# Rutgers-ECE-MML4SS/multimodal-sensor-fusion-with-attention-RajeevAtla

Hardware: AMD Instinct MI355X
Metric: HybridFusion fwd+bwd samples/sec at 1/2/4/8 MI355X; CPU-ref parity (higher is better)
Workload: dtype fp32; 1 GPU; c2: HybridFusion M=3 B=256/gpu L=128 D=128 H=128 heads=4 C=5 dropout=0.1 train, fwd+CE(ls=0.05)+bwd+clip(1.0)+AdamW; fused step (flat buffers, one hipGraph); global_batch=256, per_gpu_batch=256, seq_len=128, parallelism=dp1, graph=True, matmul_precision=highest

## Files before the change

### include/mmfusion.h

```cpp
#ifndef MMFUSION_H_
#define MMFUSION_H_

#include <stddef.h>
#include <stdint.h>

#ifdef __cplusplus
extern "C" {
#endif

#define MMF_MAX_MODALITIES 8
#define MMF_MAX_PAIRS (MMF_MAX_MODALITIES * (MMF_MAX_MODALITIES - 1))
#define MMF_MAX_HEAD_DIM 64

enum {
  MMF_PRECISION_HIGHEST = 0,
  MMF_PRECISION_MEDIUM = 1,
  MMF_PRECISION_HIGH = 2
};

enum {
  MMF_OK = 0,
  MMF_EINVAL = 1,
  MMF_ELIMIT = 2,
  MMF_EHIP = 3,
// ... 200 lines not shown
size_t mmf_transformer_encoder_saved_bytes(int32_t batch, int32_t steps, int32_t hidden, int32_t ffn,
                                           int32_t layers);
size_t mmf_transformer_encoder_workspace_bytes(int32_t batch, int32_t steps, int32_t hidden, int32_t ffn,
                                               int32_t layers, int32_t backward);
int mmf_transformer_encoder_forward(const mmf_transformer_desc* desc, const mmf_transformer_layer* params,
                                    const float* x, const int64_t* lengths, uint64_t* rng_state, void* saved,
                                    float* pooled, void* workspace, void* stream);
int mmf_transformer_encoder_backward(const mmf_transformer_desc* desc, const mmf_transformer_layer* params,
                                     const float* x, const int64_t* lengths, const void* saved,
                                     const float* dpooled, void* workspace,
                                     const mmf_transformer_layer_grad* grads, float* dx, void* stream);

int mmf_cross_entropy_ls(int32_t batch, int32_t classes, const float* logits,
                         const int64_t* labels, float smoothing, float grad_scale,
                         float* loss_out, float* dlogits, void* stream);

int mmf_adamw_step(int64_t n, float* param, const float* grad, float* exp_avg, float* exp_avg_sq,
                   int64_t* step_dev, float lr, float beta1, float beta2, float eps,
                   float weight_decay, float grad_scale, void* stream);

size_t mmf_hybrid_train_sync_bytes(const mmf_hybrid_desc* d);
int mmf_hybrid_lean_l1(const mmf_hybrid_desc* d);
int mmf_hybrid_train_status(const mmf_hybrid_desc* d, void* sync, int clear, void* stream);
int mmf_hybrid_train_step(const mmf_hybrid_desc* d, const mmf_hybrid_params* params, const float* const* x,
                          const float* mask, const int64_t* labels, float label_smoothing, float loss_scale,
                          uint64_t* rng_state, void* saved, void* workspace, void* sync, float* logits,
                          float* fusion_weights, float* loss_out, float* dlogits, const mmf_hybrid_grads* grads,
                          float* const* dx, float* clip_partial, int64_t* step_dev, const float* grad_flat,
                          int64_t grad_n, void* stream);

int mmf_hybrid_train_step_part(int part, const mmf_hybrid_desc* d, const mmf_hybrid_params* params,
                               const float* const* x, const float* mask, const int64_t* labels,
                               float label_smoothing, float loss_scale, uint64_t* rng_state, void* saved,
                               void* workspace, void* sync, float* logits, float* fusion_weights, float* loss_out,
                               float* dlogits, const mmf_hybrid_grads* grads, float* const* dx, float* clip_partial,
                               int64_t* step_dev, const float* grad_flat, int64_t grad_n, void* stream);

int mmf_adamw_step_dev(int64_t n, float* param, const float* grad, float* exp_avg, float* exp_avg_sq,
                       int64_t* step_dev, const float* lr_dev, const float* grad_coef_dev, float beta1,
                       float beta2, float eps, float weight_decay, float grad_scale, void* stream);

int mmf_clip_adamw_apply_dev(int64_t n, float* param, const float* grad, float* exp_avg, float* exp_avg_sq,
                             int64_t* step_dev, const float* lr_dev, float max_norm, float* total_norm,
                             float* clip_coef, void* workspace, float beta1, float beta2, float eps,
                             float weight_decay, float grad_scale, void* stream);

int mmf_grad_accumulate(int64_t n, const float* src, float* dst, void* stream);

size_t mmf_gemm_bf16_workspace_bytes(int32_t M, int32_t N, int32_t K, int32_t nsplit);
int mmf_gemm_bf16(int32_t M, int32_t N, int32_t K, const void* A, int32_t lda, int32_t a_kmajor, const void* B,
                  int32_t ldb, int32_t b_kmajor, const float* bias, void* C, int32_t ldc, int32_t c_bf16,
                  void* workspace, int32_t nsplit, float* bias_grad, void* stream);

size_t mmf_grad_clip_workspace_bytes(void);
int mmf_grad_clip_coef(int64_t n, const float* grad, float grad_scale, float max_norm, float* total_norm,
                       float* clip_coef, void* workspace, void* stream);

int mmf_clip_adamw_step_dev(int64_t n, float* param, const float* grad, float* exp_avg, float* exp_avg_sq,
                            int64_t* step_dev, const float* lr_dev, float max_norm, float* total_norm,
                            float* clip_coef, void* workspace, float beta1, float beta2, float eps,
                            float weight_decay, float grad_scale, void* stream);

void mmf_profile_begin(void);
size_t mmf_profile_end(char* out, size_t cap);

const char* mmf_last_error(void);
const char* mmf_version(void);

#ifdef __cplusplus
}
#endif
#endif
```

### multimodal-sensor-fusion-with-attention-rajeevatla_amd/csrc/capi.hip

```cpp
#include <cmath>
#include <map>

#include "capi_util.h"

namespace mmf {

thread_local std::string g_err;
Prof g_prof;

int fail(int code, const char* fmt, ...) {
  char buf[512];
  va_list ap;
  va_start(ap, fmt);
  vsnprintf(buf, sizeof(buf), fmt, ap);
  va_end(ap);
  g_err = buf;
  return code;
}

}

using namespace mmf;

namespace {
// ... 491 lines not shown
  hipStream_t st = (hipStream_t)stream;
  STAGE_TRY("optim.clip_adamw", launch_clip_adamw_apply(n, param, grad, exp_avg, exp_avg_sq, step_dev, lr_dev, beta1,
                                                        beta2, eps, weight_decay, grad_scale, max_norm, total_norm,
                                                        clip_coef, (const float*)workspace, st));
  return MMF_OK;
}

int mmf_grad_accumulate(int64_t n, const float* src, float* dst, void* stream) {
  if (n < 0 || (n > 0 && (!src || !dst))) return fail(MMF_EINVAL, "bad gradient-accumulate arguments");
  if ((reinterpret_cast<uintptr_t>(src) | reinterpret_cast<uintptr_t>(dst)) & 15)
    return fail(MMF_EINVAL, "gradient accumulate: buffers must be 16-byte aligned");
  hipStream_t st = (hipStream_t)stream;
  STAGE_TRY("optim.grad_accum", launch_grad_accum(n, src, dst, st));
  return MMF_OK;
}

size_t mmf_gemm_bf16_workspace_bytes(int32_t M, int32_t N, int32_t K, int32_t nsplit) {
  if (M < 1 || N < 1 || K < 1 || nsplit < 1) return 0;
  int ns = nsplit, kchunk = 0;
  split_rows(K, ns, kchunk, nsplit);
  return ((((size_t)ns * M * N * 4) + 255) & ~size_t(255)) + ((((size_t)ns * M * 4) + 255) & ~size_t(255)) + 256;
}

int mmf_gemm_bf16(int32_t M, int32_t N, int32_t K, const void* A, int32_t lda, int32_t a_kmajor, const void* B,
                  int32_t ldb, int32_t b_kmajor, const float* bias, void* C, int32_t ldc, int32_t c_bf16,
                  void* workspace, int32_t nsplit, float* bias_grad, void* stream) {
  if (M < 1 || N < 1 || K < 1 || !A || !B || !C || ldc < N || nsplit < 1)
    return fail(MMF_EINVAL, "bad bf16 GEMM arguments");
  if (a_kmajor && !b_kmajor) return fail(MMF_EINVAL, "bf16 GEMM: A k-major needs B k-major");
  if ((nsplit > 1 || bias_grad) && (!workspace || !a_kmajor || bias || c_bf16))
    return fail(MMF_EINVAL, "bf16 GEMM: split-K / bias rows need a workspace, a k-major A and an fp32 C");
  const int amode = a_kmajor ? MODE_KR : MODE_RK, bmode = b_kmajor ? MODE_KR : MODE_RK;
  hipStream_t st = (hipStream_t)stream;
  const Operand a = opnd(static_cast<const float*>(A), lda), b = opnd(static_cast<const float*>(B), ldb);
  if (nsplit == 1 && !bias_grad) {
    GemmJob j = make_job(M, N, static_cast<float*>(C), ldc, (bias ? EPI_BIAS : 0) | (c_bf16 ? EPI_BF16 : 0));
    j.g.bias = bias;
    add_src(j, a, b, K);
    if (!gemm_b16_ok(j, amode, bmode)) return fail(MMF_EINVAL, "bf16 GEMM: operand alignment / extents");
    STAGE_TRY("gemm_bf16", launch_gemm_b16(&j, 1, st, amode, bmode));
    return MMF_OK;
  }
  if (ldc != N) return fail(MMF_EINVAL, "bf16 GEMM: split-K writes a dense C (ldc == N)");
  WgradPlan wp;
  wp.split_hint = nsplit;
  Bump bw(workspace);
  plan_wgrad(wp, bw, M, N, K, a, b, static_cast<float*>(C), bias_grad, bias_grad != nullptr);
  if (!gemm_b16_ok(wp.jobs[0], amode, bmode)) return fail(MMF_EINVAL, "bf16 GEMM: operand alignment / extents");
  STAGE_TRY("gemm_bf16", launch_gemm_b16(wp.jobs.data(), 1, st, amode, bmode));
  STAGE_TRY("gemm_bf16_reduce", launch_reduce(wp.reds.data(), 1, st));
  return MMF_OK;
}

int mmf_adamw_step_dev(int64_t n, float* param, const float* grad, float* exp_avg, float* exp_avg_sq,
                       int64_t* step_dev, const float* lr_dev, const float* grad_coef_dev, float beta1,
                       float beta2, float eps, float weight_decay, float grad_scale, void* stream) {
  if (n < 0 || !param || !grad || !exp_avg || !exp_avg_sq || !step_dev || !lr_dev)
    return fail(MMF_EINVAL, "bad AdamW arguments");
  hipStream_t st = (hipStream_t)stream;
  STAGE_TRY("optim.adamw", launch_adamw(n, param, grad, exp_avg, exp_avg_sq, step_dev, 0.f, beta1, beta2, eps,
                                        weight_decay, grad_scale, st, lr_dev, grad_coef_dev));
  return MMF_OK;
}

}
```

### multimodal-sensor-fusion-with-attention-rajeevatla_amd/csrc/gemm.hip

```cpp
#include <algorithm>
#include <cstdlib>
#include <cstring>
#include <map>
#include <vector>

#include "mmf_device.h"
#include "mmf_env.h"

namespace mmf {

namespace {

constexpr int BM = 128, BN = 128, BK = 32, NT = 256;
#ifndef MMF_GEMM_DK
#define MMF_GEMM_DK 16
#endif
#ifndef MMF_GEMM_NS
#define MMF_GEMM_NS 3
#endif
constexpr int LDS_STRIDE = BM + 4;
constexpr int LDS_STRIDE_T = BM + 1;

typedef float f32x4 __attribute__((ext_vector_type(4)));

// ... 803 lines not shown
#pragma unroll
          for (int e = 0; e < 4; ++e) {
            v[e] = acc[a][b][4 * q + e] * G.alpha + bias[b];
            if (G.epi & EPI_RELU) v[e] = fmaxf(v[e], 0.f);
          }
          {
            const bool up = (x & 2) != 0;
            const float s0 = dpp<DPP_XOR2>(up ? v[0] : v[2]);
            const float s1 = dpp<DPP_XOR2>(up ? v[1] : v[3]);
            if (up) { v[0] = s0; v[1] = s1; } else { v[2] = s0; v[3] = s1; }
          }
          {
            const bool odd = (x & 1) != 0;
            const float s0 = dpp<DPP_XOR1>(odd ? v[0] : v[1]);
            const float s1 = dpp<DPP_XOR1>(odd ? v[2] : v[3]);
            if (odd) { v[0] = s0; v[2] = s1; } else { v[1] = s0; v[3] = s1; }
          }
          const int row = i0 + a * 32 + 8 * q + 4 * h + x;
          const int col = wn * 64 + b * 32 + (c & ~3);
          if (epi & EPI_ROWSCALE) {
#pragma unroll
            for (int e = 0; e < 4; ++e) v[e] *= rsc;
          }
          if (drop) {
            const uint4 rr = philox_block(rs, G.drop_site, ((uint64_t)row * (uint64_t)G.N + (uint64_t)(col & ~7)) >> 3);
#pragma unroll
            for (int e = 0; e < 4; ++e) v[e] = keep_from(rr, (col & 4) + e, thr) ? v[e] * inv_keep : 0.f;
          }
          if (epi & EPI_COLSUM) {
#pragma unroll
            for (int e = 0; e < 4; ++e) csum[b][e] += v[e];
          }
          *reinterpret_cast<f32x4*>(G.C + (int64_t)row * G.ldc + col) = f32x4{v[0], v[1], v[2], v[3]};
        }
      }
    if (epi & EPI_COLSUM) {
      float mine = 0.f;
#pragma unroll
      for (int b = 0; b < 2; ++b)
#pragma unroll
        for (int e = 0; e < 4; ++e) {
          float sv = csum[b][e];
          sv += dpp<DPP_XOR1>(sv);
          sv += dpp<DPP_XOR2>(sv);
          sv = sum_xor32(sv);
          if (b == h && e == x) mine = sv;
        }
      const int colx = wn * 64 + 32 * h + c;
      if (wm == 1) csx[colx] = mine;
      lds_barrier();
      if (wm == 0 && colx < G.N) G.colsum[(int64_t)rt * G.N + colx] = mine + csx[colx];
    }
    epi_mark = nissued;
  }
}

constexpr int WSR16_NKS = 16;
typedef __bf16 bf16x4s __attribute__((ext_vector_type(4)));

template <int WSR16_NS, int NWV = 4>
__global__ __launch_bounds__(64 * NWV, NWV == 8 ? 1 : 2) void gemm_wsr_b16_kernel(const GemmArgs args, int total_items, int K) {
  constexpr int DTILE = BM * 32 / 2;
  constexpr int PW = BM * 32 * 2 / 1024 / NWV;
  __shared__ __attribute__((aligned(16))) float ring[WSR16_NS * DTILE];
  const int t = threadIdx.x;
  const int lane = t & 63, wave = t >> 6;
  const int h = lane >> 5, c = lane & 31;
  const int wm = NWV == 8 ? wave >> 2 : wave >> 1, wn = NWV == 8 ? wave & 3 : wave & 1;
  const int nkt = K / 32, nks = K / 16;

  const int nwg = gridDim.x;
  const int item0 = (int)(((int64_t)blockIdx.x * total_items) / nwg);
  const int item1 = (int)(((int64_t)(blockIdx.x + 1) * total_items) / nwg);
  if (item0 >= item1) return;

  const int nflat = (item1 - item0) * nkt;
  auto item_group = [&](int item, int& rowtile) {
    int g = 0;
#pragma unroll
    for (int i = 1; i < GEMM_MAX_GROUPS; ++i)
      if (i < args.ngroups && item >= args.tile_off[i]) g = i;
    rowtile = item - args.tile_off[g];
    return g;
  };
  int di = item0, dk = 0, drt = 0;
  int dg = item_group(item0, drt);
  const int g_first = dg, rt_first = drt;
  auto issue = [&](int f) {
    const int slot = f % WSR16_NS;
    const GemmSrc& S = args.s[args.g[dg].src_begin];
    stage_tile_b16_nw<NWV>(ring + slot * DTILE, S.a, 0, drt * BM, args.g[dg].M, dk * 32, K, wave, lane);
    if (++dk == nkt) {
      dk = 0;
      ++di;
      ++drt;
      while (dg + 1 < args.ngroups && di >= args.tile_off[dg + 1]) { ++dg; drt = di - args.tile_off[dg]; }
    }
  };
  auto wait_ahead = [&](int ahead, bool stores_younger) {
    const int n = PW * ahead + (stores_younger ? 16 : 0);
    switch (n) {
#define MMF_WC(N) case N: asm volatile("s_waitcnt vmcnt(" #N ")" ::: "memory"); break;
      MMF_WC(0) MMF_WC(1) MMF_WC(2) MMF_WC(3) MMF_WC(4) MMF_WC(5) MMF_WC(6) MMF_WC(7) MMF_WC(8)
      MMF_WC(9) MMF_WC(10) MMF_WC(11) MMF_WC(12) MMF_WC(13) MMF_WC(14) MMF_WC(15) MMF_WC(16) MMF_WC(17)
      MMF_WC(18) MMF_WC(19) MMF_WC(20) MMF_WC(21) MMF_WC(22) MMF_WC(23) MMF_WC(24) MMF_WC(25) MMF_WC(26)
      MMF_WC(27) MMF_WC(28) MMF_WC(29) MMF_WC(30) MMF_WC(31) MMF_WC(32) MMF_WC(33) MMF_WC(34) MMF_WC(35)
// ... 509 lines not shown
hipError_t launch_wsr(const GemmJob* jobs, int njobs, hipStream_t st, uint64_t* rng_advance, int bmode, float drop_p,
                      const RngSnap* rng) {
  for (int done = 0; done < njobs;) {
    GemmArgs args;
    memset(&args, 0, sizeof(args));
    args.amode = MODE_RK;
    args.bmode = bmode;
    args.drop_p = drop_p;
    args.rng = rng;
    args.rng_advance = rng_advance;
    rng_advance = nullptr;
    int ng = 0, items = 0;
    double fl = 0.0, by = 0.0;
    while (done < njobs && ng < GEMM_MAX_GROUPS) {
      GemmGroup g = jobs[done].g;
      g.nbatch = 1;
      g.src_begin = ng;
      g.src_count = 1;
      args.s[ng] = jobs[done].src[0];
      args.tile_off[ng] = items;
      args.g[ng++] = g;
      items += g.M / BM;
      fl += 2.0 * g.M * g.N * jobs[done].src[0].K;
      by += 4.0 * ((double)g.M + g.N) * jobs[done].src[0].K + 4.0 * g.M * g.N;
      ++done;
    }
    args.ngroups = ng;
    const int K = args.s[0].K;
    const int grid = std::min(items, 2 * cu_count());
    const int pr = math_mode();
    bool ext = bmode != MODE_RK;
    for (int i = 0; i < ng; ++i) ext = ext || (args.g[i].epi & ~(EPI_BIAS | EPI_RELU)) != 0;
#define MMF_WSR_LAUNCH(BFV, EXTV, NAME)                                             \
  {                                                                                 \
    ProfLaunch prof_(st, NAME, fl, by);                                             \
    mmf_launch((gemm_wsr_kernel<BFV, EXTV>), dim3(grid), dim3(NT), 0, st, args, items, K); \
  }
    if (ext) {
      if (pr == 2) MMF_WSR_LAUNCH(2, true, "gemm_wsr_kernel<2, true>")
      else if (pr == 1) MMF_WSR_LAUNCH(1, true, "gemm_wsr_kernel<1, true>")
      else MMF_WSR_LAUNCH(0, true, "gemm_wsr_kernel<0, true>")
    } else {
      if (pr == 2) MMF_WSR_LAUNCH(2, false, "gemm_wsr_kernel<2>")
      else if (pr == 1) MMF_WSR_LAUNCH(1, false, "gemm_wsr_kernel<1>")
      else MMF_WSR_LAUNCH(0, false, "gemm_wsr_kernel<0>")
    }
#undef MMF_WSR_LAUNCH
    hipError_t e = hipGetLastError();
    if (e != hipSuccess) return e;
  }
  return hipSuccess;
}

}

int device_cu_count() { return cu_count(); }

hipError_t launch_gemm(const GemmJob* jobs_in, int njobs, int amode, int bmode, float drop_p,
                       const RngSnap* rng, hipStream_t st, uint64_t* rng_advance) {
  for (int i = 0; i < njobs; ++i)
    if ((jobs_in[i].g.epi & EPI_BF16) &&
        (!job_fast(jobs_in[i], amode, bmode) || jobs_in[i].g.nbatch > 1 || (jobs_in[i].g.epi & EPI_PARTIAL)))
      return hipErrorInvalidValue;
  {
    bool wsr = njobs > 0;
    for (int i = 0; i < njobs && wsr; ++i)
      wsr = job_wsr(jobs_in[i], amode, bmode) && jobs_in[i].src[0].K == jobs_in[0].src[0].K && !jobs_in[i].chain;
    if (wsr && !switch_set<SW_NO_WSR>()) return launch_wsr(jobs_in, njobs, st, rng_advance, bmode, drop_p, rng);
  }
  struct AdvanceLeft {
    uint64_t*& adv;
    hipStream_t st;
    hipError_t finish(hipError_t e) { return (e == hipSuccess && adv) ? launch_rng_advance(adv, st) : e; }
  } left{rng_advance, st};
  std::vector<GemmJob> rest;
  {
    SmallSlabArgs sa;
    memset(&sa, 0, sizeof(sa));
    int total = 0;
    double fl = 0.0, by = 0.0;
    auto flush = [&]() -> hipError_t {
      if (sa.ngroups == 0) return hipSuccess;
      sa.off[sa.ngroups] = total;
      ProfLaunch prof_(st, "small_slab_kernel", fl, by);
      mmf_launch(small_slab_kernel, dim3((8 * total + 255) / 256), dim3(256), 0, st, sa);
      memset(&sa, 0, sizeof(sa));
      total = 0; fl = by = 0.0;
      return hipGetLastError();
    };
    for (int i = 0; i < njobs; ++i) {
      const GemmJob& J = jobs_in[i];
      if (job_fast(J, amode, bmode) || !job_small_slab(J, amode, bmode) || J.chain) {
        rest.push_back(J);
        continue;
      }
      GemmGroup g = J.g;
      if (g.nbatch < 1) g.nbatch = 1;
      sa.g[sa.ngroups] = g;
      sa.s[sa.ngroups] = J.src[0];
      sa.off[sa.ngroups] = total;
      total += g.nbatch * g.nsplit * g.M * (g.N + (g.part_db ? 1 : 0));
      fl += 2.0 * g.nbatch * g.M * g.N * J.src[0].K;
      by += 4.0 * g.nbatch * ((double)g.M + g.N) * J.src[0].K + 4.0 * g.nbatch * g.nsplit * g.M * g.N;
      if (++sa.ngroups == GEMM_MAX_GROUPS)
        if (hipError_t e = flush()) return e;
    }
    if (hipError_t e = flush()) return e;
    if (rest.empty()) return left.finish(hipSuccess);
    jobs_in = rest.data();
    njobs = (int)rest.size();
  }
  auto chain_ok = [&](const GemmJob& J) {
    const GemmJob* C = J.chain;
    if (!C || amode != MODE_RK) return false;
    const GemmGroup &a = J.g, &b = C->g;
    if (!job_fast(J, amode, bmode) || !job_fast(*C, amode, bmode)) return false;
    if ((a.epi & (EPI_PARTIAL | EPI_BF16)) || (b.epi & EPI_PARTIAL) || a.nbatch > 1 || b.nbatch > 1) return false;
    if (a.N > BN || b.N > BN || b.M != a.M || C->nsrc != 1) return false;
    const GemmSrc& x = C->src[0];
    return x.a.ptr == a.C && x.a.ld == a.ldc && x.K == a.N && x.a.row_div == 1 && x.a.seg_stride == 0;
  };
// ... 478 lines not shown
```

### multimodal-sensor-fusion-with-attention-rajeevatla_amd/csrc/mmf_env.h

```cpp
#pragma once

#include <cstdint>
#include <cstdlib>
#include <cstring>
#include <unistd.h>

namespace mmf {

#define MMF_SWITCHES(X)        \
  X(PSTORE, 1, 0)              \
  X(NO_LONG_FUSED, 1, 0)       \
  X(NO_FUSED_BWD, 1, 0)        \
  X(NO_BF16_QK, 1, 0)          \
  X(NO_GEMM_B16, 1, 0)         \
  X(QK_CAT, 1, 0)              \
  X(NO_DQK_B16, 1, 0)          \
  X(NO_PROJ_B16, 1, 0)         \
  X(NO_PCOL, 1, 0)             \
  X(NO_POOLE, 1, 0)            \
  X(POOLE_FLAT, 1, 0)          \
  X(NO_L1_LEAN, 1, 0)          \
  X(WGRAD_SPLIT_CAP, 1, 0)     \
  X(NO_SIDE_STREAM, 1, 0)      \
  X(SIDE_STREAM, 1, 0)         \
  X(KW_SERIAL, 1, 0)           \
  X(KW_FUSED, 1, 0)            \
  X(NO_KW_FUSED, 1, 0)         \
  X(NO_GATE_B16, 1, 0)         \
  X(POOL_PER_PAIR, 1, 0)       \
  X(TAIL_S, 1, 0)              \
  X(DX_CHAIN, 0, 0)            \
  X(GEMM_ILV, 0, 0)            \
  X(NO_WSR, 0, 0)              \
  X(NO_WSR16, 0, 0)            \
  X(WSR16_NS, 0, 0)            \
  X(L1_POLL_BOUND, 0, 0)       \
  X(TAIL_HEAD_GEMV, 0, 0)      \
  X(WSR_EPI, 0, 1)             \
  X(TAIL_GEMV, 0, 1)           \
  X(POOL_VALU, 0, 1)           \
  X(WSR16_W4, 0, 1)            \
  X(GEMM_NO_WIDE, 0, 1)        \
  X(GEMM_WIDE_DZ, 0, 1)        \
  X(LONG_FWD_W8, 0, 1)

enum Switch {
#define X(name, plan, once) SW_##name,
  MMF_SWITCHES(X)
#undef X
  SW_COUNT
};

struct SwitchInfo { const char* name; bool plan, once; };
constexpr SwitchInfo kSwitches[SW_COUNT] = {
#define X(name, plan, once) {"MMF_" #name, plan != 0, once != 0},
    MMF_SWITCHES(X)
#undef X
};

template <Switch S>
inline const char* switch_value() {
  static_assert(!kSwitches[S].once, "a once-per-process switch is only set or unset");
  return getenv(kSwitches[S].name);
}

template <Switch S>
inline bool switch_set() {
  if constexpr (kSwitches[S].once) {
    static const bool set = getenv(kSwitches[S].name) != nullptr;
    return set;
  } else {
    return getenv(kSwitches[S].name) != nullptr;
  }
}

inline uint32_t plan_fingerprint() {
  uint32_t sum = 0;
  for (char** e = environ; e && *e; ++e) {
    const char* s = *e;
    if (std::strncmp(s, "MMF_", 4) != 0) continue;
    for (const SwitchInfo& k : kSwitches) {
      if (!k.plan) continue;
      const size_t n = std::strlen(k.name);
      if (std::strncmp(s, k.name, n) != 0 || s[n] != '=') continue;
      uint32_t h = 2166136261u;
// ... 10 lines not shown
```

### multimodal-sensor-fusion-with-attention-rajeevatla_amd/mmf_native.py

```python

from __future__ import annotations

import ctypes
import os
from ctypes import c_float, c_int32, c_int64, c_size_t, c_void_p, POINTER
from typing import Optional

import torch

MAX_MODALITIES = 8
MAX_PAIRS = MAX_MODALITIES * (MAX_MODALITIES - 1)
MAX_HEAD_DIM = 64
PRECISION_HIGHEST = 0
PRECISION_MEDIUM = 1
PRECISION_HIGH = 2


def matmul_precision() -> int:
    mode = torch.get_float32_matmul_precision()
    return {"medium": PRECISION_MEDIUM, "high": PRECISION_HIGH}.get(mode, PRECISION_HIGHEST)

_HERE = os.path.dirname(os.path.abspath(__file__))
LIB_PATH = os.environ.get("MMF_LIB_PATH") or os.path.join(_HERE, "csrc", "libmmfusion.so")

EXPORTED_SYMBOLS = (
    "mmf_hybrid_saved_bytes", "mmf_hybrid_workspace_bytes", "mmf_hybrid_forward",
    "mmf_hybrid_backward", "mmf_hybrid_train_sync_bytes", "mmf_hybrid_train_status", "mmf_hybrid_train_step",
    "mmf_hybrid_train_step_part", "mmf_hybrid_plan_flags", "mmf_hybrid_saved_region",
    "mmf_adaptive_weights_workspace_bytes", "mmf_adaptive_weights",
    "mmf_adaptive_weights_backward",
    "mmf_cma_saved_bytes", "mmf_cma_workspace_bytes", "mmf_cma_forward", "mmf_cma_backward",
    "mmf_cross_entropy_ls", "mmf_adamw_step", "mmf_adamw_step_dev", "mmf_grad_clip_workspace_bytes",
    "mmf_grad_clip_coef", "mmf_clip_adamw_step_dev", "mmf_clip_adamw_apply_dev", "mmf_grad_accumulate", "mmf_gemm_bf16_workspace_bytes", "mmf_gemm_bf16", "mmf_hybrid_lean_l1", "mmf_profile_begin", "mmf_profile_end",
    "mmf_last_error", "mmf_version",
    "mmf_attention_pool_workspace_bytes", "mmf_attention_pool_forward", "mmf_attention_pool_backward",
    "mmf_late_fusion_workspace_bytes", "mmf_late_fusion_forward", "mmf_late_fusion_backward",
    "mmf_gather_chunks",
    "mmf_lstm_sync_bytes", "mmf_lstm_forward", "mmf_lstm_backward",
    "mmf_gru_sync_bytes", "mmf_gru_forward", "mmf_gru_backward",
    "mmf_mc_reduce", "mmf_hybrid_mc_forward", "mmf_temperature_nll_workspace_bytes", "mmf_temperature_nll",
    "mmf_uncertainty_fusion_forward", "mmf_uncertainty_fusion_backward",
    "mmf_conv_encoder_workspace_bytes", "mmf_conv_encoder_forward", "mmf_conv_encoder_backward",
    "mmf_transformer_encoder_saved_bytes", "mmf_transformer_encoder_workspace_bytes",
    "mmf_transformer_encoder_forward", "mmf_transformer_encoder_backward",
    "mmf_hybrid_sweep_workspace_bytes", "mmf_hybrid_sweep_forward", "mmf_confusion_accumulate",
)


class Linear(ctypes.Structure):
    _fields_ = [("w", c_void_p), ("b", c_void_p)]


class HybridDesc(ctypes.Structure):
    _fields_ = [
        ("batch", c_int32), ("num_modalities", c_int32), ("hidden", c_int32),
        ("num_heads", c_int32), ("num_classes", c_int32),
        ("seq_len", c_int32 * MAX_MODALITIES), ("in_dim", c_int32 * MAX_MODALITIES),
        ("num_pairs", c_int32),
        ("pair_q", c_int32 * MAX_PAIRS), ("pair_k", c_int32 * MAX_PAIRS),
        ("dropout", c_float), ("training", c_int32), ("return_attention", c_int32),
        ("matmul_precision", c_int32),
        ("plan_flags", ctypes.c_uint32), ("saved_capacity", ctypes.c_uint64),
        ("workspace_capacity", ctypes.c_uint64),
    ]


class HybridParams(ctypes.Structure):
    _fields_ = [
        ("proj", Linear * MAX_MODALITIES),
        ("q", Linear * MAX_PAIRS), ("k", Linear * MAX_PAIRS),
        ("v", Linear * MAX_PAIRS), ("o", Linear * MAX_PAIRS),
        ("gate", Linear * MAX_MODALITIES),
        ("cls1", Linear), ("cls2", Linear),
    ]


HybridGrads = HybridParams


class CmaDesc(ctypes.Structure):
    _fields_ = [
        ("batch", c_int32), ("lq", c_int32), ("lk", c_int32), ("query_dim", c_int32),
        ("key_dim", c_int32), ("hidden", c_int32), ("num_heads", c_int32),
        ("mask_mode", c_int32), ("dropout", c_float), ("training", c_int32),
        ("matmul_precision", c_int32),
    ]


class CmaParams(ctypes.Structure):
    _fields_ = [("q", Linear), ("k", Linear), ("v", Linear), ("o", Linear)]


CmaGrads = CmaParams

TRANSFORMER_MAX_LAYERS = 8
TRANSFORMER_LAYER_FIELDS = ("in_proj_w", "in_proj_b", "out_proj_w", "out_proj_b", "linear1_w", "linear1_b",
                            "linear2_w", "linear2_b", "norm1_w", "norm1_b", "norm2_w", "norm2_b")


class TransformerDesc(ctypes.Structure):
    _fields_ = [
        ("batch", c_int32), ("steps", c_int32), ("hidden", c_int32), ("ffn", c_int32), ("layers", c_int32),
        ("training", c_int32), ("dropout", c_float), ("eps", c_float),
    ]


class TransformerLayer(ctypes.Structure):
    _fields_ = [(name, c_void_p) for name in TRANSFORMER_LAYER_FIELDS]


TransformerLayerGrad = TransformerLayer

_LIB: Optional[ctypes.CDLL] = None


def lib() -> ctypes.CDLL:
    global _LIB
    if _LIB is not None:
        return _LIB
    if not os.path.exists(LIB_PATH):
        raise RuntimeError(
            f"mmfusion: HIP library not found at {LIB_PATH}. Build it with "
            f"`make -C {os.path.join(_HERE, 'csrc')}` (hipcc --offload-arch=gfx950). "
            "There is no CPU fallback.")
    L = ctypes.CDLL(LIB_PATH)
    vp, sz = c_void_p, c_size_t
    L.mmf_hybrid_saved_bytes.argtypes = [POINTER(HybridDesc)]
    L.mmf_hybrid_saved_bytes.restype = sz
    L.mmf_hybrid_workspace_bytes.argtypes = [POINTER(HybridDesc)]
    L.mmf_hybrid_workspace_bytes.restype = sz
    L.mmf_hybrid_plan_flags.argtypes = []
    L.mmf_hybrid_plan_flags.restype = ctypes.c_uint32
    L.mmf_hybrid_saved_region.argtypes = [POINTER(HybridDesc), c_int32, c_int32, POINTER(ctypes.c_uint64),
                                          POINTER(ctypes.c_uint64)]
    L.mmf_hybrid_saved_region.restype = c_int32
    L.mmf_hybrid_forward.argtypes = [POINTER(HybridDesc), POINTER(HybridParams), vp, vp, vp, vp,
                                     vp, vp, vp, vp]
    L.mmf_hybrid_forward.restype = c_int32
    L.mmf_hybrid_backward.argtypes = [POINTER(HybridDesc), POINTER(HybridParams), vp, vp, vp, vp,
                                      vp, POINTER(HybridGrads), vp, vp]
    L.mmf_hybrid_backward.restype = c_int32
    L.mmf_hybrid_train_sync_bytes.argtypes = [POINTER(HybridDesc)]
    L.mmf_hybrid_train_sync_bytes.restype = sz
    L.mmf_hybrid_lean_l1.argtypes = [POINTER(HybridDesc)]
    L.mmf_hybrid_lean_l1.restype = c_int32
    L.mmf_hybrid_train_status.argtypes = [POINTER(HybridDesc), vp, c_int32, vp]
    L.mmf_hybrid_train_status.restype = c_int32
    L.mmf_hybrid_train_step.argtypes = [POINTER(HybridDesc), POINTER(HybridParams), vp, vp, vp, c_float, c_float,
                                        vp, vp, vp, vp, vp, vp, vp, vp, POINTER(HybridGrads), vp, vp, vp, vp,
                                        c_int64, vp]
    L.mmf_hybrid_train_step.restype = c_int32
    L.mmf_hybrid_train_step_part.argtypes = [c_int32] + L.mmf_hybrid_train_step.argtypes
    L.mmf_hybrid_train_step_part.restype = c_int32
    L.mmf_adaptive_weights_workspace_bytes.argtypes = [c_int32, c_int32, c_int32]
    L.mmf_adaptive_weights_workspace_bytes.restype = sz
    L.mmf_adaptive_weights.argtypes = [c_int32, c_int32, c_int32, vp, vp, vp, vp, vp, vp]
    L.mmf_adaptive_weights.restype = c_int32
    L.mmf_adaptive_weights_backward.argtypes = [c_int32, c_int32, c_int32, vp, vp, vp, vp, vp, vp, vp, vp]
    L.mmf_adaptive_weights_backward.restype = c_int32
    L.mmf_cma_saved_bytes.argtypes = [POINTER(CmaDesc)]
    L.mmf_cma_saved_bytes.restype = sz
    L.mmf_cma_workspace_bytes.argtypes = [POINTER(CmaDesc)]
    L.mmf_cma_workspace_bytes.restype = sz
    L.mmf_cma_forward.argtypes = [POINTER(CmaDesc), POINTER(CmaParams), vp, vp, vp, vp, vp, vp,
                                  vp, vp, vp]
    L.mmf_cma_forward.restype = c_int32
    L.mmf_cma_backward.argtypes = [POINTER(CmaDesc), POINTER(CmaParams), vp, vp, vp, vp, vp, vp,
                                   vp, POINTER(CmaGrads), vp, vp, vp, vp]
    L.mmf_cma_backward.restype = c_int32
    L.mmf_cross_entropy_ls.argtypes = [c_int32, c_int32, vp, vp, c_float, c_float, vp, vp, vp]
    L.mmf_cross_entropy_ls.restype = c_int32
    L.mmf_adamw_step.argtypes = [c_int64, vp, vp, vp, vp, vp, c_float, c_float, c_float, c_float,
                                 c_float, c_float, vp]
    L.mmf_adamw_step.restype = c_int32
    L.mmf_adamw_step_dev.argtypes = [c_int64, vp, vp, vp, vp, vp, vp, vp, c_float, c_float, c_float, c_float,
                                     c_float, vp]
    L.mmf_adamw_step_dev.restype = c_int32
    L.mmf_grad_clip_workspace_bytes.argtypes = []
    L.mmf_grad_clip_workspace_bytes.restype = c_size_t
    L.mmf_grad_clip_coef.argtypes = [c_int64, vp, c_float, c_float, vp, vp, vp, vp]
    L.mmf_grad_clip_coef.restype = c_int32
    L.mmf_clip_adamw_step_dev.argtypes = [c_int64, vp, vp, vp, vp, vp, vp, c_float, vp, vp, vp, c_float, c_float,
                                          c_float, c_float, c_float, vp]
    L.mmf_clip_adamw_step_dev.restype = c_int32
    L.mmf_clip_adamw_apply_dev.argtypes = [c_int64, vp, vp, vp, vp, vp, vp, c_float, vp, vp, vp, c_float, c_float,
                                           c_float, c_float, c_float, vp]
    L.mmf_clip_adamw_apply_dev.restype = c_int32
    L.mmf_grad_accumulate.argtypes = [c_int64, vp, vp, vp]
    L.mmf_grad_accumulate.restype = c_int32
    L.mmf_gemm_bf16_workspace_bytes.argtypes = [c_int32, c_int32, c_int32, c_int32]
    L.mmf_gemm_bf16_workspace_bytes.restype = sz
    L.mmf_gemm_bf16.argtypes = [c_int32, c_int32, c_int32, vp, c_int32, c_int32, vp, c_int32, c_int32, vp, vp,
                                c_int32, c_int32, vp, c_int32, vp, vp]
    L.mmf_gemm_bf16.restype = c_int32
    L.mmf_profile_begin.argtypes = []
    L.mmf_profile_begin.restype = None
    L.mmf_profile_end.argtypes = [ctypes.c_char_p, c_size_t]
    L.mmf_profile_end.restype = c_size_t
    L.mmf_attention_pool_workspace_bytes.argtypes = [c_int32, c_int32]
    L.mmf_attention_pool_workspace_bytes.restype = sz
    L.mmf_attention_pool_forward.argtypes = [c_int32, c_int32, c_int32, vp, vp, vp, vp, vp, vp, vp]
    L.mmf_attention_pool_forward.restype = c_int32
    L.mmf_attention_pool_backward.argtypes = [c_int32, c_int32, c_int32, vp, vp, vp, vp, vp, vp, vp, vp, vp]
    L.mmf_attention_pool_backward.restype = c_int32
    L.mmf_late_fusion_workspace_bytes.argtypes = [c_int32, c_int32]
    L.mmf_late_fusion_workspace_bytes.restype = sz
    L.mmf_late_fusion_forward.argtypes = [c_int32, c_int32, c_int32, vp, vp, vp, vp, vp, vp]
    L.mmf_late_fusion_forward.restype = c_int32
    L.mmf_late_fusion_backward.argtypes = [c_int32, c_int32, c_int32, vp, vp, vp, vp, vp, vp, vp, vp, vp]
    L.mmf_late_fusion_backward.restype = c_int32
    L.mmf_gather_chunks.argtypes = [vp, c_int64, c_int32, vp, vp, c_int32, c_int32, c_int32, vp, vp, vp, c_int32,
                                     vp, vp, vp]
    L.mmf_gather_chunks.restype = c_int32
    for cell in ("lstm", "gru"):
        sync_bytes = getattr(L, f"mmf_{cell}_sync_bytes")
        sync_bytes.argtypes, sync_bytes.restype = [c_int32, c_int32], c_size_t
        for way in ("forward", "backward"):
            fn = getattr(L, f"mmf_{cell}_{way}")
            fn.argtypes, fn.restype = [c_int32] * 4 + [vp] * 8, c_int32
    L.mmf_mc_reduce.argtypes = [c_int32, c_int32, c_int32, vp, vp, vp, vp, vp]
    L.mmf_mc_reduce.restype = c_int32
    L.mmf_hybrid_mc_forward.argtypes = [POINTER(HybridDesc), POINTER(HybridParams), vp, vp, vp, c_int32, vp, vp, vp,
                                        vp, vp, vp, vp]
    L.mmf_hybrid_mc_forward.restype = c_int32
    L.mmf_temperature_nll_workspace_bytes.argtypes = [c_int64]
    L.mmf_temperature_nll_workspace_bytes.restype = sz
    L.mmf_temperature_nll.argtypes = [c_int64, c_int32, vp, vp, vp, vp, vp, vp, vp]
    L.mmf_temperature_nll.restype = c_int32
    L.mmf_uncertainty_fusion_forward.argtypes = [c_int32, c_int32, c_int32, vp, vp, vp, c_float, vp, vp, vp]
    L.mmf_uncertainty_fusion_forward.restype = c_int32
    L.mmf_uncertainty_fusion_backward.argtypes = [c_int32, c_int32, c_int32, vp, vp, vp, c_float, vp, vp, vp, vp]
    L.mmf_uncertainty_fusion_backward.restype = c_int32
    L.mmf_conv_encoder_workspace_bytes.argtypes = [c_int32] * 5
    L.mmf_conv_encoder_workspace_bytes.restype = sz
    L.mmf_conv_encoder_forward.argtypes = ([c_int32] * 5 + [vp] * 7 + [c_float] + [vp] * 6 + [c_float]
                                           + [vp] * 7)
    L.mmf_conv_encoder_forward.restype = c_int32
    L.mmf_conv_encoder_backward.argtypes = [c_int32] * 5 + [vp] * 19
    L.mmf_conv_encoder_backward.restype = c_int32
    L.mmf_transformer_encoder_saved_bytes.argtypes = [c_int32] * 5
    L.mmf_transformer_encoder_saved_bytes.restype = sz
    L.mmf_transformer_encoder_workspace_bytes.argtypes = [c_int32] * 6
    L.mmf_transformer_encoder_workspace_bytes.restype = sz
    L.mmf_transformer_encoder_forward.argtypes = [POINTER(TransformerDesc), vp] + [vp] * 7
    L.mmf_transformer_encoder_forward.restype = c_int32
    L.mmf_transformer_encoder_backward.argtypes = [POINTER(TransformerDesc), vp] + [vp] * 8
    L.mmf_transformer_encoder_backward.restype = c_int32
# ... 71 lines not shown
```

Measured before the change: 272,500 samples/s.

## Add persistent streaming fp32 GEMM kernel for narrow-N short-K jobs

Adds a persistent gemm_stream_kernel that walks 64-row half tiles across all groups with a 3-stage async global-to-LDS ring, so loads for the next tile are in flight while the current tile's epilogue (bias, relu, rowscale, dropout, colsum) runs. It is enabled by default and takes eligible jobs (N<=128, K<=128, dense RK/KR operands) that fall past the WSR path, aiming to cut per-tile prologue and launch-tail costs. It also exposes an mmf_gemm_f32 C API with a Python binding. The risks are fiddly vmcnt accounting and colsum pairing across half tiles, and lower per-tile MFMA efficiency from the smaller M tile.

```diff
diff --git a/include/mmfusion.h b/include/mmfusion.h
--- a/include/mmfusion.h
+++ b/include/mmfusion.h
@@ -276,6 +276,21 @@
                   int32_t ldb, int32_t b_kmajor, const float* bias, void* C, int32_t ldc, int32_t c_bf16,
                   void* workspace, int32_t nsplit, float* bias_grad, void* stream);
 
+typedef struct mmf_gemm_f32_job {
+  int32_t M, N, K;
+  const float* A; int32_t lda;
+  const float* B; int32_t ldb;
+  const float* bias;
+  int32_t relu;
+  const float* rowscale; int32_t rs_div, rs_stride, rs_off;
+  int32_t drop; uint32_t drop_site;
+  float* colsum;
+  float* C; int32_t ldc;
+  int32_t nsplit;
+} mmf_gemm_f32_job;
+int mmf_gemm_f32(const mmf_gemm_f32_job* jobs, int32_t njobs, int32_t b_kmajor, float drop_p, const uint64_t* rng,
+                 int32_t precision, void* stream);
+
 size_t mmf_grad_clip_workspace_bytes(void);
 int mmf_grad_clip_coef(int64_t n, const float* grad, float grad_scale, float max_norm, float* total_norm,
                        float* clip_coef, void* workspace, void* stream);
diff --git a/multimodal-sensor-fusion-with-attention-rajeevatla_amd/csrc/capi.hip b/multimodal-sensor-fusion-with-attention-rajeevatla_amd/csrc/capi.hip
--- a/multimodal-sensor-fusion-with-attention-rajeevatla_amd/csrc/capi.hip
+++ b/multimodal-sensor-fusion-with-attention-rajeevatla_amd/csrc/capi.hip
@@ -567,6 +567,39 @@
   return MMF_OK;
 }
 
+int mmf_gemm_f32(const mmf_gemm_f32_job* jobs, int32_t njobs, int32_t b_kmajor, float drop_p, const uint64_t* rng,
+                 int32_t precision, void* stream) {
+  if (!jobs || njobs < 1 || drop_p < 0.f || drop_p >= 1.f) return fail(MMF_EINVAL, "bad fp32 GEMM arguments");
+  mmf::MathScope math_(precision);
+  hipStream_t st = (hipStream_t)stream;
+  std::vector<GemmJob> js;
+  for (int i = 0; i < njobs; ++i) {
+    const mmf_gemm_f32_job& q = jobs[i];
+    if (q.M < 1 || q.N < 1 || q.K < 1 || !q.A || !q.B || !q.C || q.nsplit < 1 || q.ldc < q.N)
+      return fail(MMF_EINVAL, "bad fp32 GEMM job");
+    if (q.rowscale && q.rs_div < 1) return fail(MMF_EINVAL, "fp32 GEMM: rs_div < 1");
+    if (q.nsplit > 1 && (q.bias || q.relu || q.rowscale || q.drop || q.colsum || q.ldc != q.N))
+      return fail(MMF_EINVAL, "fp32 GEMM: split-K slabs take no epilogue and a dense C");
+    GemmJob j = make_job(q.M, q.N, q.C, q.ldc,
+                         (q.bias ? EPI_BIAS : 0) | (q.relu ? EPI_RELU : 0) | (q.rowscale ? EPI_ROWSCALE : 0) |
+                             (q.drop ? EPI_DROP : 0) | (q.colsum ? EPI_COLSUM : 0) | (q.nsplit > 1 ? EPI_PARTIAL : 0));
+    j.g.bias = q.bias;
+    j.g.rowscale = q.rowscale; j.g.rs_div = q.rowscale ? q.rs_div : 1; j.g.rs_stride = q.rs_stride; j.g.rs_off = q.rs_off;
+    j.g.drop_site = q.drop_site;
+    if (q.colsum) j.g.colsum = q.colsum;
+    if (q.nsplit > 1) {
+      j.g.nsplit = q.nsplit;
+      j.g.kchunk = ((q.K + q.nsplit - 1) / q.nsplit + 31) & ~31;
+      if ((int64_t)(q.nsplit - 1) * j.g.kchunk >= q.K) return fail(MMF_EINVAL, "fp32 GEMM: an empty split-K slab");
+    }
+    add_src(j, opnd(q.A, q.lda), opnd(q.B, q.ldb), q.K);
+    js.push_back(j);
+  }
+  STAGE_TRY("gemm_f32", launch_gemm(js.data(), (int)js.size(), MODE_RK, b_kmajor ? MODE_KR : MODE_RK, drop_p,
+                                    reinterpret_cast<const RngSnap*>(rng), st));
+  return MMF_OK;
+}
+
 int mmf_adamw_step_dev(int64_t n, float* param, const float* grad, float* exp_avg, float* exp_avg_sq,
                        int64_t* step_dev, const float* lr_dev, const float* grad_coef_dev, float beta1,
                        float beta2, float eps, float weight_decay, float grad_scale, void* stream) {
diff --git a/multimodal-sensor-fusion-with-attention-rajeevatla_amd/csrc/gemm.hip b/multimodal-sensor-fusion-with-attention-rajeevatla_amd/csrc/gemm.hip
--- a/multimodal-sensor-fusion-with-attention-rajeevatla_amd/csrc/gemm.hip
+++ b/multimodal-sensor-fusion-with-attention-rajeevatla_amd/csrc/gemm.hip
@@ -879,6 +879,221 @@
       if (wm == 0 && colx < G.N) G.colsum[(int64_t)rt * G.N + colx] = mine + csx[colx];
     }
     epi_mark = nissued;
+  }
+}
+
+constexpr int ST_BM = 64, ST_DK = 16, ST_NS = 3;
+constexpr int ST_A = ST_BM * ST_DK;
+constexpr int ST_STAGE = ST_A + BN * ST_DK;
+constexpr int ST_DMA = 3;
+
+__device__ __forceinline__ float scale_then_add(float a, float s, float b) {
+#pragma clang fp contract(off)
+  const float m = a * s;
+  return m + b;
+}
+
+__device__ __forceinline__ void wait_vm(int n) {
+  switch (n) {
+#define MMF_WC(N) case N: asm volatile("s_waitcnt vmcnt(" #N ")" ::: "memory"); break;
+    MMF_WC(1) MMF_WC(2) MMF_WC(3) MMF_WC(4) MMF_WC(5) MMF_WC(6) MMF_WC(7) MMF_WC(8) MMF_WC(9)
+    MMF_WC(10) MMF_WC(11) MMF_WC(12) MMF_WC(13) MMF_WC(14) MMF_WC(15) MMF_WC(16) MMF_WC(17)
+    MMF_WC(18) MMF_WC(19) MMF_WC(20) MMF_WC(21) MMF_WC(22) MMF_WC(23) MMF_WC(24)
+#undef MMF_WC
+    default: asm volatile("s_waitcnt vmcnt(0)" ::: "memory"); break;
+  }
+}
+
+__host__ __device__ inline int stream_run(int b, int nwg, int units) { return (int)(((int64_t)b * units) / nwg); }
+
+template <int BMODE, int BF>
+__global__ __launch_bounds__(NT, 3) void gemm_stream_kernel(const GemmArgs args, int total_units, int K) {
+  __shared__ __attribute__((aligned(16))) float lds[ST_NS * ST_STAGE + 4 * BN];
+  float* const ring = lds;
+  float* const csx = lds + ST_NS * ST_STAGE;
+  const int t = threadIdx.x;
+  const int lane = t & 63, wave = __builtin_amdgcn_readfirstlane(t >> 6);
+  const int h = lane >> 5, c = lane & 31;
+  const int wm = wave >> 1, wn = wave & 1;
+  const int nkt = K / ST_DK;
+
+  RngSnap rs{0, 0};
+  const float p = args.drop_p;
+  const float inv_keep = p < 1.f ? 1.f / (1.f - p) : 0.f;
+  const uint32_t thr = p16(p);
+  if (p > 0.f && args.rng) rs = *args.rng;
+  if (args.rng_advance && blockIdx.x == 0 && threadIdx.x == 0) args.rng_advance[1] += 1;
+  const int u0 = stream_run(blockIdx.x, gridDim.x, total_units);
+  const int u1 = stream_run(blockIdx.x + 1, gridDim.x, total_units);
+  if (u0 >= u1) return;
+
+  auto live = [&](int g, int hf) { return g < args.ngroups && args.tile_off[g] + (hf >> 1) < u1; };
+  auto adv = [&](int& g, int& hf) {
+    if (++hf * ST_BM >= args.g[g].M) { ++g; hf = 0; }
+  };
+  int g0 = 0;
+#pragma unroll
+  for (int i = 1; i < GEMM_MAX_GROUPS; ++i)
+    if (i < args.ngroups && u0 >= args.tile_off[i]) g0 = i;
+  const int hf0 = 2 * (u0 - args.tile_off[g0]);
+
+  int dg = g0, dhf = hf0, dk = 0, dslot = 0, nissued = 0;
+  bool dlive = true;
+  auto issue = [&]() {
+    const GemmSrc& S = args.s[dg];
+    float* stg = ring + dslot * ST_STAGE;
+    {
+      const int row = wave * 16 + (lane >> 2);
+      const int slot = (lane & 3) ^ swz<ST_DK>(row);
+      const float* src = S.a.ptr + (int64_t)(dhf * ST_BM + row) * S.a.ld + dk * ST_DK + 4 * slot;
+      __builtin_amdgcn_global_load_lds((const void*)src,
+                                       (__attribute__((address_space(3))) void*)(stg + wave * 256), 16, 0, 0);
+    }
+    stage_tile<BMODE, ST_DK>(stg + ST_A, S.b, 0, 0, args.g[dg].N, dk * ST_DK, K, wave, lane);
+    dslot = dslot == ST_NS - 1 ? 0 : dslot + 1;
+    ++nissued;
+    if (++dk == nkt) {
+      dk = 0;
+      adv(dg, dhf);
+      dlive = live(dg, dhf);
+    }
+  };
+  for (int q = 0; q < ST_NS - 1 && dlive; ++q) issue();
+
+  int f = 0, slot = 0, st1 = 0, st2 = 0;
+  int cur_g = -1;
+  float bias[2] = {0.f, 0.f};
+  for (int g = g0, hf = hf0; live(g, hf); adv(g, hf)) {
+    const GemmGroup& G = args.g[g];
+    if (g != cur_g) {
+      cur_g = g;
+#pragma unroll
+      for (int b = 0; b < 2; ++b) {
+        const int col = wn * 64 + b * 32 + c;
+        bias[b] = (col < G.N && (G.epi & EPI_BIAS)) ? G.bias[col] : 0.f;
+      }
+      __builtin_amdgcn_s_waitcnt(0x0F70);
+    }
+    f32x16 acc[2];
+#pragma unroll
+    for (int b = 0; b < 2; ++b)
+#pragma unroll
+      for (int r = 0; r < 16; ++r) acc[b][r] = 0.f;
+
+    for (int kt = 0; kt < nkt; ++kt) {
+      wait_vm(ST_DMA * (nissued - f - 1) + st1 + st2);
+      lds_barrier();
+      if (dlive) issue();
+      const float* At = ring + slot * ST_STAGE;
+      const float* Bt = At + ST_A;
+      if constexpr (BF != 0) {
+        float av[8], bv[2][8];
+#pragma unroll
+        for (int j = 0; j < 2; ++j) {
+          const f32x4 fa = frag<MODE_RK, ST_DK>(At, wm * 32 + c, j, h);
+#pragma unroll
+          for (int s = 0; s < 4; ++s) av[4 * j + s] = fa[s];
+#pragma unroll
+          for (int b = 0; b < 2; ++b) {
+            const f32x4 fb = frag<BMODE, ST_DK>(Bt, wn * 64 + b * 32 + c, j, h);
+#pragma unroll
+            for (int s = 0; s < 4; ++s) bv[b][4 * j + s] = fb[s];
+          }
+        }
+#pragma unroll
+        for (int b = 0; b < 2; ++b) acc[b] = mfma_k16<BF>(av, bv[b], acc[b]);
+      } else {
+#pragma unroll
+        for (int j = 0; j < 2; ++j) {
+          const f32x4 af = frag<MODE_RK, ST_DK>(At, wm * 32 + c, j, h);
+          f32x4 bf[2];
+#pragma unroll
+          for (int b = 0; b < 2; ++b) bf[b] = frag<BMODE, ST_DK>(Bt, wn * 64 + b * 32 + c, j, h);
+#pragma unroll
+          for (int s = 0; s < 4; ++s)
+#pragma unroll
+            for (int b = 0; b < 2; ++b) acc[b] = mfma32(af[s], bf[b][s], acc[b]);
+        }
+      }
+      ++f;
+      slot = slot == ST_NS - 1 ? 0 : slot + 1;
+      st2 = st1;
+      st1 = 0;
+    }
+    const int x = c & 3;
+    const int i0 = hf * ST_BM + wm * 32;
+    const int epi = G.epi;
+    const bool drop = (epi & EPI_DROP) && p > 0.f;
+    float rsc = 1.f;
+    if (epi & EPI_ROWSCALE)
+      rsc = ((const __attribute__((address_space(4))) float*)G.rowscale)[(hf * ST_BM / G.rs_div) * G.rs_stride + G.rs_off];
+    float csum[2][4] = {{0.f, 0.f, 0.f, 0.f}, {0.f, 0.f, 0.f, 0.f}};
+    int nst = 0;
+#pragma unroll
+    for (int b = 0; b < 2; ++b) {
+      const int col = wn * 64 + b * 32 + (c & ~3);
+      if (wn * 64 + b * 32 < G.N) nst += 4;
+#pragma unroll
+      for (int q = 0; q < 4; ++q) {
+        float v[4];
+#pragma unroll
+        for (int e = 0; e < 4; ++e) {
+          v[e] = scale_then_add(acc[b][4 * q + e], G.alpha, bias[b]);
+          if (epi & EPI_RELU) v[e] = fmaxf(v[e], 0.f);
+        }
+        {
+          const bool up = (x & 2) != 0;
+          const float s0 = dpp<DPP_XOR2>(up ? v[0] : v[2]);
+          const float s1 = dpp<DPP_XOR2>(up ? v[1] : v[3]);
+          if (up) { v[0] = s0; v[1] = s1; } else { v[2] = s0; v[3] = s1; }
+        }
+        {
+          const bool odd = (x & 1) != 0;
+          const float s0 = dpp<DPP_XOR1>(odd ? v[0] : v[1]);
+          const float s1 = dpp<DPP_XOR1>(odd ? v[2] : v[3]);
+          if (odd) { v[0] = s0; v[2] = s1; } else { v[1] = s0; v[3] = s1; }
+        }
+        const int row = i0 + 8 * q + 4 * h + x;
+        if (epi & EPI_ROWSCALE) {
+#pragma unroll
+          for (int e = 0; e < 4; ++e) v[e] *= rsc;
+        }
+        if (drop) {
+          const uint4 rr = philox_block(rs, G.drop_site, ((uint64_t)row * (uint64_t)G.N + (uint64_t)(col & ~7)) >> 3);
+#pragma unroll
+          for (int e = 0; e < 4; ++e) v[e] = keep_from(rr, (col & 4) + e, thr) ? v[e] * inv_keep : 0.f;
+        }
+        if (epi & EPI_COLSUM) {
+#pragma unroll
+          for (int e = 0; e < 4; ++e) csum[b][e] += v[e];
+        }
+        if (col < G.N) *reinterpret_cast<f32x4*>(G.C + (int64_t)row * G.ldc + col) = f32x4{v[0], v[1], v[2], v[3]};
+      }
+    }
+    if (epi & EPI_COLSUM) {
+      float mine = 0.f;
+#pragma unroll
+      for (int b = 0; b < 2; ++b)
+#pragma unroll
+        for (int e = 0; e < 4; ++e) {
+          float sv = csum[b][e];
+          sv += dpp<DPP_XOR1>(sv);
+          sv += dpp<DPP_XOR2>(sv);
+          sv = sum_xor32(sv);
+          if (b == h && e == x) mine = sv;
+        }
+      csx[((hf & 1) * 2 + wm) * BN + wn * 64 + 32 * h + c] = mine;
+      if ((hf & 1) || (hf + 1) * ST_BM >= G.M) {
+        lds_barrier();
+        if (t < G.N) {
+          float s = csx[t] + csx[BN + t];
+          if (hf & 1) s = (s + csx[2 * BN + t]) + csx[3 * BN + t];
+          G.colsum[(int64_t)(hf >> 1) * G.N + t] = s;
+        }
+        if (wave * 64 < G.N) nst += 1;
+      }
+    }
+    st1 = nst;
   }
 }
 
@@ -1494,6 +1709,92 @@
   return hipSuccess;
 }
 
+bool job_stream(const GemmJob& J, int amode, int bmode) {
+  const GemmGroup& g = J.g;
+  if (amode != MODE_RK || (bmode != MODE_RK && bmode != MODE_KR) || J.nsrc != 1 || g.nbatch > 1 || J.chain) return false;
+  if (g.epi & ~(EPI_BIAS | EPI_RELU | EPI_DROP | EPI_COLSUM | EPI_ROWSCALE)) return false;
+  if ((g.epi & EPI_ROWSCALE) && (g.rs_div <= 0 || g.rs_div % ST_BM != 0 || !g.rowscale)) return false;
+  if ((g.epi & EPI_COLSUM) && !g.colsum) return false;
+  if ((g.epi & EPI_BIAS) && !g.bias) return false;
+  const GemmSrc& s = J.src[0];
+  return g.N >= 8 && g.N <= BN && g.N % 8 == 0 && g.M >= ST_BM && g.M % ST_BM == 0 && s.K % ST_DK == 0 &&
+         s.K >= ST_DK && s.K <= 128 && g.seg_rows == 0 && s.a.row_div == 1 && s.b.row_div == 1 &&
+         s.a.seg_stride == 0 && s.b.seg_stride == 0 && s.a.ld % 4 == 0 && aligned16(s.a.ptr) && s.b.ld % 4 == 0 &&
+         aligned16(s.b.ptr) && g.ldc % 4 == 0 && aligned16(g.C);
+}
+
+bool gemm_stream_on() {
+  const char* e = switch_value<SW_GEMM_STREAM>();
+  if (!e || !e[0]) return true;
+  return e[0] != '0';
+}
+
+template <typename F>
+int stream_grid(F kernel, int units) {
+  static const int occ = [&] {
+    int n = 0;
+    return hipOccupancyMaxActiveBlocksPerMultiprocessor(&n, kernel, NT, 0) == hipSuccess && n >= 1 ? n : 1;
+  }();
+  int grid = std::min(units, occ * cu_count());
+  if (const char* e = switch_value<SW_GEMM_STREAM_GRID>()) {
+    const int cap = atoi(e);
+    if (cap >= 1) grid = std::min(grid, cap);
+  }
+  return std::max(grid, 1);
+}
+
+hipError_t launch_stream(const GemmJob* jobs, int njobs, hipStream_t st, uint64_t* rng_advance, int bmode, float drop_p,
+                         const RngSnap* rng) {
+  for (int done = 0; done < njobs;) {
+    GemmArgs args;
+    memset(&args, 0, sizeof(args));
+    args.amode = MODE_RK;
+    args.bmode = bmode;
+    args.drop_p = drop_p;
+    args.rng = rng;
+    args.rng_advance = rng_advance;
+    rng_advance = nullptr;
+    int ng = 0, units = 0;
+    double fl = 0.0, by = 0.0;
+    while (done < njobs && ng < GEMM_MAX_GROUPS) {
+      GemmGroup g = jobs[done].g;
+      g.nbatch = 1;
+      g.src_begin = ng;
+      g.src_count = 1;
+      g.chain = 0;
+      args.s[ng] = jobs[done].src[0];
+      args.tile_off[ng] = units;
+      args.g[ng++] = g;
+      units += (g.M + BM - 1) / BM;
+      fl += 2.0 * g.M * g.N * jobs[done].src[0].K;
+      by += 4.0 * ((double)g.M + g.N) * jobs[done].src[0].K + 4.0 * g.M * g.N;
+      ++done;
+    }
+    args.ngroups = ng;
+    const int K = args.s[0].K;
+    const int pr = math_mode();
+#define MMF_STREAM_LAUNCH(BMV, BFV, NAME)                                                         \
+  {                                                                                               \
+    const int grid = stream_grid(gemm_stream_kernel<BMV, BFV>, units);                            \
+    ProfLaunch prof_(st, NAME, fl, by);                                                           \
+    mmf_launch((gemm_stream_kernel<BMV, BFV>), dim3(grid), dim3(NT), 0, st, args, units, K);      \
+  }
+    if (bmode == MODE_KR) {
+      if (pr == 2) MMF_STREAM_LAUNCH(MODE_KR, 2, "gemm_stream_kernel<1, 2>")
+      else if (pr == 1) MMF_STREAM_LAUNCH(MODE_KR, 1, "gemm_stream_kernel<1, 1>")
+      else MMF_STREAM_LAUNCH(MODE_KR, 0, "gemm_stream_kernel<1, 0>")
+    } else {
+      if (pr == 2) MMF_STREAM_LAUNCH(MODE_RK, 2, "gemm_stream_kernel<0, 2>")
+      else if (pr == 1) MMF_STREAM_LAUNCH(MODE_RK, 1, "gemm_stream_kernel<0, 1>")
+      else MMF_STREAM_LAUNCH(MODE_RK, 0, "gemm_stream_kernel<0, 0>")
+    }
+#undef MMF_STREAM_LAUNCH
+    hipError_t e = hipGetLastError();
+    if (e != hipSuccess) return e;
+  }
+  return hipSuccess;
+}
+
 }
 
 int device_cu_count() { return cu_count(); }
@@ -1509,6 +1810,12 @@
     for (int i = 0; i < njobs && wsr; ++i)
       wsr = job_wsr(jobs_in[i], amode, bmode) && jobs_in[i].src[0].K == jobs_in[0].src[0].K && !jobs_in[i].chain;
     if (wsr && !switch_set<SW_NO_WSR>()) return launch_wsr(jobs_in, njobs, st, rng_advance, bmode, drop_p, rng);
+  }
+  {
+    bool stream = njobs > 0 && gemm_stream_on();
+    for (int i = 0; i < njobs && stream; ++i)
+      stream = job_stream(jobs_in[i], amode, bmode) && jobs_in[i].src[0].K == jobs_in[0].src[0].K;
+    if (stream) return launch_stream(jobs_in, njobs, st, rng_advance, bmode, drop_p, rng);
   }
   struct AdvanceLeft {
     uint64_t*& adv;
diff --git a/multimodal-sensor-fusion-with-attention-rajeevatla_amd/csrc/mmf_env.h b/multimodal-sensor-fusion-with-attention-rajeevatla_amd/csrc/mmf_env.h
--- a/multimodal-sensor-fusion-with-attention-rajeevatla_amd/csrc/mmf_env.h
+++ b/multimodal-sensor-fusion-with-attention-rajeevatla_amd/csrc/mmf_env.h
@@ -29,8 +29,10 @@
   X(NO_GATE_B16, 1, 0)         \
   X(POOL_PER_PAIR, 1, 0)       \
   X(TAIL_S, 1, 0)              \
+  X(GEMM_STREAM, 1, 0)         \
   X(DX_CHAIN, 0, 0)            \
   X(GEMM_ILV, 0, 0)            \
+  X(GEMM_STREAM_GRID, 0, 0)    \
   X(NO_WSR, 0, 0)              \
   X(NO_WSR16, 0, 0)            \
   X(WSR16_NS, 0, 0)            \
diff --git a/multimodal-sensor-fusion-with-attention-rajeevatla_amd/mmf_native.py b/multimodal-sensor-fusion-with-attention-rajeevatla_amd/mmf_native.py
--- a/multimodal-sensor-fusion-with-attention-rajeevatla_amd/mmf_native.py
+++ b/multimodal-sensor-fusion-with-attention-rajeevatla_amd/mmf_native.py
@@ -31,7 +31,7 @@
     "mmf_adaptive_weights_backward",
     "mmf_cma_saved_bytes", "mmf_cma_workspace_bytes", "mmf_cma_forward", "mmf_cma_backward",
     "mmf_cross_entropy_ls", "mmf_adamw_step", "mmf_adamw_step_dev", "mmf_grad_clip_workspace_bytes",
-    "mmf_grad_clip_coef", "mmf_clip_adamw_step_dev", "mmf_clip_adamw_apply_dev", "mmf_grad_accumulate", "mmf_gemm_bf16_workspace_bytes", "mmf_gemm_bf16", "mmf_hybrid_lean_l1", "mmf_profile_begin", "mmf_profile_end",
+    "mmf_grad_clip_coef", "mmf_clip_adamw_step_dev", "mmf_clip_adamw_apply_dev", "mmf_grad_accumulate", "mmf_gemm_bf16_workspace_bytes", "mmf_gemm_bf16", "mmf_gemm_f32", "mmf_hybrid_lean_l1", "mmf_profile_begin", "mmf_profile_end",
     "mmf_last_error", "mmf_version",
     "mmf_attention_pool_workspace_bytes", "mmf_attention_pool_forward", "mmf_attention_pool_backward",
     "mmf_late_fusion_workspace_bytes", "mmf_late_fusion_forward", "mmf_late_fusion_backward",
@@ -110,6 +110,21 @@
 
 
 TransformerLayerGrad = TransformerLayer
+
+
+class GemmF32Job(ctypes.Structure):
+    _fields_ = [
+        ("M", c_int32), ("N", c_int32), ("K", c_int32),
+        ("A", c_void_p), ("lda", c_int32),
+        ("B", c_void_p), ("ldb", c_int32),
+        ("bias", c_void_p),
+        ("relu", c_int32),
+        ("rowscale", c_void_p), ("rs_div", c_int32), ("rs_stride", c_int32), ("rs_off", c_int32),
+        ("drop", c_int32), ("drop_site", ctypes.c_uint32),
+        ("colsum", c_void_p),
+        ("C", c_void_p), ("ldc", c_int32),
+        ("nsplit", c_int32),
+    ]
 
 _LIB: Optional[ctypes.CDLL] = None
 
@@ -193,6 +208,8 @@
     L.mmf_gemm_bf16.argtypes = [c_int32, c_int32, c_int32, vp, c_int32, c_int32, vp, c_int32, c_int32, vp, vp,
                                 c_int32, c_int32, vp, c_int32, vp, vp]
     L.mmf_gemm_bf16.restype = c_int32
+    L.mmf_gemm_f32.argtypes = [POINTER(GemmF32Job), c_int32, c_int32, c_float, vp, c_int32, vp]
+    L.mmf_gemm_f32.restype = c_int32
     L.mmf_profile_begin.argtypes = []
     L.mmf_profile_begin.restype = None
     L.mmf_profile_end.argtypes = [ctypes.c_char_p, c_size_t]
```

Result: no change. 273,700 samples/s (median of 6 runs) (+0.4%).
